# roshanprabhakar/flexflow-train

Hardware: AMD Instinct MI355X
Metric: samples_per_sec_whole_node (higher is better)
Workload: dtype bf16; 1 GPU; model=bert-large, global_batch=128, batch_per_gpu=128, seq_len=512, parallelism=dp1, layers=24, hidden=1024, heads=16, vocab=30522, optimizer=adamw, hipgraph=True, native_replay=True

## Files before the change

csrc/kernels/attention.hip:

```cpp
#include <cstdlib>
#include <type_traits>

#include "kernels.h"
#include "mfma.h"

namespace ffk {

template <class T>
struct TensorViewT {
  T* p;
  int64_t sb, ss, sh;
  __device__ __forceinline__ T* row(int b, int s, int h) const { return p + b * sb + static_cast<int64_t>(s) * ss + h * sh; }
};
using TensorView = TensorViewT<const bf16>;
using OutView = TensorViewT<bf16>;

struct AttnParams {
  TensorView q, k, v, o, dout;
  OutView o_out, dq, dk, dv;
  float* lse;
  float* delta;
  float *dbq, *dbk, *dbv;
  int64_t db_ld;
  int B, H, Sq, Sk;
// ... 164 lines not shown

__device__ __forceinline__ float bfi_sel(unsigned m, float a, float b) {
  float r;
  asm("v_bfi_b32 %0, %1, %2, %3" : "=v"(r) : "v"(m), "v"(a), "v"(b));
  return r;
}
template <int DT>
__device__ __forceinline__ void bias_partial(const f32x16 (&acc)[DT], float mul, float* row, int lane) {
  constexpr int NV = 16 * DT;
  float v[NV];
#pragma unroll
  for (int dt = 0; dt < DT; ++dt)
#pragma unroll
    for (int r = 0; r < 16; ++r) v[dt * 16 + r] = acc[dt][r];
#pragma unroll
  for (int st = 0; st < 5; ++st) {
    const int o = 16 >> st, c = NV >> st;
    const unsigned m = (lane & o) ? ~0u : 0u;
#pragma unroll
    for (int i = 0; i < c / 2; ++i) {
      const float send = bfi_sel(m, v[i], v[i + c / 2]);
      const float keep = bfi_sel(m, v[i + c / 2], v[i]);
      v[i] = keep + __shfl_xor(send, o, 64);
    }
  }
  const int h = lane >> 5;
#pragma unroll
  for (int t = 0; t < NV / 32; ++t) {
    const int k = (lane & 31) * (NV / 32) + t, dt = k >> 4, r = k & 15;
    row[dt * 32 + acc_row(r) + 4 * h] = v[t] * mul;
  }
}

template <int D, bool CAUSAL, bool DROP, bool VARLEN, bool PACKED, bool BIAS, bool GQA = false>
__global__ __launch_bounds__(256, (BIAS && D == 128 ? 1 : 2)) void attn_fwd_kernel(AttnParams P) {
  constexpr int KS = D / 16;
  constexpr int DT = D / 32;
  constexpr int KV = 64;
  constexpr int TILE_BYTES = KV * D * 2;
  __shared__ __attribute__((aligned(16))) unsigned char smem[4 * TILE_BYTES];

  const int lane = threadIdx.x & 63, wave = threadIdx.x >> 6, h = lane >> 5;
  int bh = blockIdx.x, qb = gridDim.y - 1 - blockIdx.y;
  if (!CAUSAL) attn_head_block(bh, qb);
  const int b = bh / P.H, hh = bh % P.H;
  const int hk = kv_head<GQA>(P, hh);
  [[maybe_unused]] int pn = b, ps = 0, plen = 0;
  if constexpr (PACKED) {
    const Segment sg = segment_of(P, b);
    pn = sg.n, ps = sg.start, plen = sg.len;
  }
  const int q_blk = qb * 128;
  const int qw = q_blk + wave * 32;
  const int q = qw + (lane & 31);
  const bool q_ok = PACKED ? q < plen : q < P.Sq;
  const int Skl = PACKED ? plen : key_len<VARLEN>(P, b);
  [[maybe_unused]] const int Sql = PACKED ? plen : query_len<VARLEN>(P, b);
  const bool q_live = VARLEN ? q < Sql : q_ok;
  if constexpr (VARLEN) {
    if (q_blk >= Sql) {
      if constexpr (!PACKED) {
        if (q_ok) {
          store_zero_rows<D>(P.o_out.row(b, q, hh), h);
          if (h == 0) P.lse[static_cast<int64_t>(bh) * P.Sq + q] = -INFINITY;
        }
      }
// ... 624 lines not shown
            }
            dv[dt] = mfma32(da, pf, dv[dt]);
            dk[dt] = mfma32(qa, sf, dk[dt]);
          }
        }
        prio_lo(P);
      }
    }
    if (has_next) {
      unsigned char* nxt = smem + ((t + 1 - t0) & 1) * STAGE;
      ql.store(nxt);
      dl.store(nxt + TILE_BYTES);
      park_scalars(nxt);
    }
    __syncthreads();
    if constexpr (GQA) tq = tq_n, hq = hq_n;
  }
  float vmul = 1.f;
  if constexpr (DROP) vmul = P.drop_rs;
  if (P.db_ld) {
    if (kw < P.Sk) {
      const int64_t roff = (static_cast<int64_t>(b) * ((P.Sk + 31) / 32) + kw / 32) * P.db_ld + hh * D;
      if (P.dbk) bias_partial<DT>(dk, P.scale, P.dbk + roff, lane);
      if (P.dbv) bias_partial<DT>(dv, vmul, P.dbv + roff, lane);
    }
  } else {
    if (P.dbk) bias_colsum<DT>(dk, P.scale, P.dbk + hh * D, lane);
    if (P.dbv) bias_colsum<DT>(dv, vmul, P.dbv + hh * D, lane);
  }
  store_rows16<DT>(P.dk.row(pn, ps + key, hh), dk, P.scale, h, k_st);
  store_rows16<DT>(P.dv.row(pn, ps + key, hh), dv, vmul, h, k_st);
}

__global__ __launch_bounds__(512, 1) void attn_bwd_onepass_kernel(AttnParams P, float* __restrict__ ws) {
  constexpr int D = 64, KS = D / 16, DT = D / 32, QT = 64, KB = 256, NT = 512;
  constexpr int TILE_BYTES = QT * D * 2;
  constexpr int STAGE = 2 * TILE_BYTES + 2 * QT * 4;
  constexpr int KIMG_BYTES = KB * D * 2, DS_BYTES = KB * QT * 2;
  __shared__ __attribute__((aligned(16))) unsigned char smem[2 * STAGE + KIMG_BYTES + 2 * DS_BYTES];
  unsigned char* const Kimg = smem + 2 * STAGE;
  unsigned char* const dSimg = Kimg + KIMG_BYTES;
  const int lane = threadIdx.x & 63, wave = __builtin_amdgcn_readfirstlane(threadIdx.x >> 6), h = lane >> 5;
  const int bh = blockIdx.x, b = bh / P.H, hh = bh % P.H;
  const int n_q_tiles = (P.Sq + QT - 1) / QT;
  const int n_kb = (P.Sk + KB - 1) / KB;
  const int w4 = wave & 3, dq_par = wave >> 2, dq_q = (w4 & 1) * 32, dq_d = (w4 >> 1) * 32;
  const int srow = threadIdx.x >> 3, sch = threadIdx.x & 7;

  TileLoader<D, QT, NT> ql, dl, ol;
  float nls = 0.f;
  bool nok = false;
  auto fetch = [&](int q0) {
    ql.load(P.q, b, hh, q0, P.Sq);
    dl.load(P.dout, b, hh, q0, P.Sq);
    ol.load(P.o, b, hh, q0, P.Sq);
    nok = q0 + srow < P.Sq;
    if (nok && sch == 0) nls = P.lse[static_cast<int64_t>(bh) * P.Sq + q0 + srow];
  };
  auto park = [&](unsigned char* stage) {
    ql.store(stage);
    dl.store(stage + TILE_BYTES);
    float part = 0.f;
#pragma unroll
    for (int e = 0; e < 8; ++e) part += bf2f(ol.reg[0][e]) * bf2f(dl.reg[0][e]);
#pragma unroll
    for (int o = 1; o < 8; o <<= 1) part += __shfl_xor(part, o, 64);
    if (sch == 0) {
      float* ls = reinterpret_cast<float*>(stage + 2 * TILE_BYTES);
      ls[srow] = nok ? -nls * P.inv_scale_log2 : -INFINITY;
      ls[QT + srow] = -part;
    }
  };

  for (int kb = 0; kb < n_kb; ++kb) {
    const int k_blk = kb * KB;
    const int kl_ = wave * 32 + (lane & 31);
    const int kw = k_blk + wave * 32, key = k_blk + kl_;
    const bool k_ok = key < P.Sk;
    const bool last_kb = kb == n_kb - 1;
    bf16x8 vf[KS];
#pragma unroll
    for (int ks = 0; ks < KS; ++ks) {
      vf[ks] = k_ok ? *reinterpret_cast<const bf16x8*>(P.v.row(b, key, hh) + ks * 16 + 8 * h) : bf16x8{};
    }
    {
      int r0 = srow;
      asm volatile("" : "+v"(r0));
      const bf16* kp = P.k.row(b, k_blk + r0, hh) + sch * 8;
      bf16x8 kr[KB / 64];
#pragma unroll
      for (int i = 0; i < KB / 64; ++i)
        kr[i] = k_blk + r0 + 64 * i < P.Sk ? *reinterpret_cast<const bf16x8*>(kp + 64 * i * P.k.ss) : bf16x8{};
      int q0 = 0;
      asm volatile("" : "+s"(q0));
      fetch(q0);
#pragma unroll
      for (int i = 0; i < KB / 64; ++i) *reinterpret_cast<bf16x8*>(Kimg + lds_off<D>(r0 + 64 * i, sch)) = kr[i];
    }
    park(smem);
    __syncthreads();

    f32x16 dk[DT], dv[DT];
#pragma unroll
    for (int dt = 0; dt < DT; ++dt) dk[dt] = dv[dt] = f32x16{};

    auto dq_tile = [&](int t) {
      const unsigned char* dS = dSimg + (t & 1) * DS_BYTES;
      float* wp = ws + ((static_cast<int64_t>(bh) * n_q_tiles + t) * 4 + w4) * 1024 + lane * 4;
      f32x16 acc[1] = {f32x16{}};
      const int i16 = lane & 15, colq = 16 * ((lane >> 4) & 1) + 4 * (i16 & 3), ra = 8 * h + (i16 >> 2);
      const int ck = dq_d + colq, cs = dq_q + colq;
      const unsigned char* ka = Kimg + img_off<D * 2>(ra, ck >> 3) + (ck & 7) * 2;
      const unsigned char* kb_ = Kimg + img_off<D * 2>(ra + 4, ck >> 3) + (ck & 7) * 2;
      const unsigned char* sa = dS + img_off<QT * 2>(ra, cs >> 3) + (cs & 7) * 2;
      const unsigned char* sb = dS + img_off<QT * 2>(ra + 4, cs >> 3) + (cs & 7) * 2;
      auto product = [&] {
        prio_hi(P);
#pragma unroll 4
        for (int k0 = 0; k0 < KB; k0 += 16) {
          const int o = k0 * 128;
          acc[0] = mfma32(cat44(lds_tr(ka, o), lds_tr(kb_, o)), cat44(lds_tr(sa, o), lds_tr(sb, o)), acc[0]);
        }
        prio_lo(P);
      };
      if (kb > 0) {
        f32x4 prev[4];
#pragma unroll
        for (int g = 0; g < 4; ++g) prev[g] = *reinterpret_cast<const f32x4*>(wp + g * 256);
        product();
#pragma unroll
        for (int g = 0; g < 4; ++g)
#pragma unroll
          for (int e = 0; e < 4; ++e) acc[0][4 * g + e] += prev[g][e];
      } else {
        product();
      }
      if (last_kb) {
        const int q = t * QT + dq_q + (lane & 31);
        store_rows16<1>(P.dq.row(b, q, hh) + dq_d, acc, P.scale, h, q < P.Sq);
      } else {
#pragma unroll
        for (int g = 0; g < 4; ++g) {
          f32x4 w;
#pragma unroll
          for (int e = 0; e < 4; ++e) w[e] = acc[0][4 * g + e];
          *reinterpret_cast<f32x4*>(wp + g * 256) = w;
        }
      }
    };

    for (int t = 0; t <= n_q_tiles; ++t) {
      const int q0 = t * QT;
      unsigned char* stage = smem + (t & 1) * STAGE;
      const unsigned char* Qt = stage;
      const unsigned char* Dt = stage + TILE_BYTES;
      const float* ls = reinterpret_cast<const float*>(stage + 2 * TILE_BYTES);
      const float* ds = ls + QT;
      unsigned char* dSw = dSimg + (t & 1) * DS_BYTES;
      fetch(q0 + QT);
      const bool need_mask = (q0 + QT > P.Sq) || (kw + 31 >= P.Sk);
      if (t < n_q_tiles) {
#pragma unroll
        for (int qt = 0; qt < 2; ++qt) {
          f32x16 s, dp;
          bf16x8 qa[KS], da[KS], kf[KS], tda[2][DT], tqa[2][DT];
#pragma unroll
          for (int ks = 0; ks < KS; ++ks) {
            const int off = lds_off<D>(qt * 32 + (lane & 31), 2 * ks + h);
            qa[ks] = lds_read16(Qt, off);
            da[ks] = lds_read16(Dt, off);
            kf[ks] = lds_read16(Kimg, lds_off<D>(kl_, 2 * ks + h));
          }
// ... 18 lines not shown
          if (need_mask) {
#pragma unroll
            for (int r = 0; r < 16; ++r) {
              const int qq = q0 + qt * 32 + acc_row(r) + 4 * h;
              float pv = fexp2(s[r] * P.scale_log2);
              if (qq >= P.Sq || !k_ok) pv = 0.f;
              s[r] = pv;
              dp[r] = pv * dp[r];
            }
          } else {
#pragma unroll
            for (int r = 0; r < 16; ++r) {
              const float pv = fexp2(s[r] * P.scale_log2);
              s[r] = pv;
              dp[r] = pv * dp[r];
            }
          }
          prio_hi(P);
#pragma unroll
          for (int st = 0; st < 2; ++st) {
            const bf16x8 pf = acc_to_frag(s, st), sf = acc_to_frag(dp, st);
            if (st == 0) {
#pragma unroll
              for (int dt = 0; dt < DT; ++dt) {
                tda[1][dt] = tr_frag<D>(Dt, qt * 32 + 16, dt, lane);
                tqa[1][dt] = tr_frag<D>(Qt, qt * 32 + 16, dt, lane);
              }
            }
#pragma unroll
            for (int g2 = 0; g2 < 2; ++g2) {
              bf16x4 w;
#pragma unroll
              for (int e = 0; e < 4; ++e) w[e] = sf[4 * g2 + e];
              *reinterpret_cast<bf16x4*>(dSw + img_off<QT * 2>(kl_, qt * 4 + 2 * st + g2) + 8 * h) = w;
            }
#pragma unroll
            for (int dt = 0; dt < DT; ++dt) {
              dv[dt] = mfma32(tda[st][dt], pf, dv[dt]);
              dk[dt] = mfma32(tqa[st][dt], sf, dk[dt]);
            }
          }
          prio_lo(P);
        }
      }
      park(smem + ((t + 1) & 1) * STAGE);
      if (t > 0 && ((t - 1) & 1) == dq_par) dq_tile(t - 1);
      __syncthreads();
    }

    store_rows16<DT>(P.dk.row(b, key, hh), dk, P.scale, h, k_ok);
    store_rows16<DT>(P.dv.row(b, key, hh), dv, 1.f, h, k_ok);
  }
}

__global__ void attn_segment_offsets_kernel(const int32_t* __restrict__ seg_lens, int32_t* __restrict__ seg_off, int N,
                                            int M, int T, int max_seqlen) {
  const int n = blockIdx.x * blockDim.x + threadIdx.x;
  if (n >= N) return;
  int start = 0;
  for (int m = 0; m < M; ++m) {
    const int64_t i = static_cast<int64_t>(n) * M + m;
    const int len = min(max(seg_lens[i], 0), min(max_seqlen, T - start));
    seg_off[2 * i] = start;
    seg_off[2 * i + 1] = len;
    start += len;
  }
}

__global__ __launch_bounds__(256) void attn_pack_tail_kernel(OutView a, OutView b, OutView c, float* __restrict__ lse,
                                                              const int32_t* __restrict__ seg_off, int M, int T, int H,
                                                              int D) {
  constexpr int ROWS = 16;
  const int n = blockIdx.y, row0 = blockIdx.x * ROWS;
  const int64_t last = (static_cast<int64_t>(n) * M + (M - 1)) * 2;
  const int tail = min(max(seg_off[last] + seg_off[last + 1], 0), T);
  if (row0 + ROWS <= tail) return;
  const int cpr = H * (D / 8);
  for (int i = threadIdx.x; i < ROWS * cpr; i += blockDim.x) {
    const int r = row0 + i / cpr, ch = i % cpr, hh = ch / (D / 8), d = (ch % (D / 8)) * 8;
    if (r < tail || r >= T) continue;
    const u32x4t z = {0u, 0u, 0u, 0u};
    if (a.p) *reinterpret_cast<u32x4t*>(a.row(n, r, hh) + d) = z;
    if (b.p) *reinterpret_cast<u32x4t*>(b.row(n, r, hh) + d) = z;
    if (c.p) *reinterpret_cast<u32x4t*>(c.row(n, r, hh) + d) = z;
  }
// ... 142 lines not shown
      constexpr int DD = decltype(d)::value;
      constexpr bool CC = decltype(c)::value, DR = decltype(dr)::value, VL = decltype(vl)::value;
      if constexpr (!DR && !VL) {
        if (P.G > 1) {
          hipLaunchKernelGGL((attn_fwd_kernel<DD, CC, false, false, false, false, true>), grid, block, 0, st, P);
          return;
        }
      }
      if constexpr (VL) {
        if (packed) {
          hipLaunchKernelGGL((attn_fwd_kernel<DD, CC, DR, true, true, false>), grid, block, 0, st, P);
          return;
        }
      }
      if constexpr (!CC && !VL) {
        if (P.bias) {
          hipLaunchKernelGGL((attn_fwd_kernel<DD, false, DR, false, false, true>), grid, block, 0, st, P);
          return;
        }
      }
      hipLaunchKernelGGL((attn_fwd_kernel<DD, CC, DR, VL, false, false>), grid, block, 0, st, P);
    });
  });
  if (packed) launch_pack_tail(P, P.o_out, OutView{}, OutView{}, P.lse, B, D, st);
  FFK_LAUNCH_CHECK("attention_fwd");
}

static bool onepass_eligible(int Sk, int D, bool causal, bool extras) {
  if (D != 64 || causal || Sk > 512 || extras) return false;
  const char* oe = getenv("FFK_ATTN_BWD_ONEPASS");
  return oe ? atoi(oe) != 0 : true;
}

int64_t attention_bwd_workspace(int B, int H, int Sq, int Sk, int D, bool causal, bool dbias, bool varlen) {
  if (!onepass_eligible(Sk, D, causal, dbias || varlen) || Sk <= 256) return 0;
  return static_cast<int64_t>(B) * H * ((Sq + 63) / 64) * 64 * 64;
}

int attention_bwd(const AttnTensors& t, int B, int H, int Sq, int Sk, int D, float scale, bool causal,
                  hipStream_t st, float* ws) {
  AttnParams P = make_params(t, B, H, Sq, Sk, D, scale, causal);
  const bool packed = P.seg_off != nullptr;
  const bool drop = P.drop_thr != 0, varlen = P.kv_lens || P.q_lens || packed;
  if (onepass_eligible(Sk, D, causal, t.dbq || t.dbk || t.dbv || drop || varlen || P.bias || P.G > 1) &&
      (Sk <= 256 || ws)) {
    hipLaunchKernelGGL(attn_bwd_onepass_kernel, dim3(static_cast<unsigned>(B * H)), dim3(512), 0, st, P, ws);
    FFK_LAUNCH_CHECK("attention_bwd");
    return 1;
  }
  const unsigned nq = static_cast<unsigned>((Sq + 127) / 128), nk = static_cast<unsigned>((Sk + 127) / 128);
  const unsigned nbh = static_cast<unsigned>(packed ? B * P.M * H : B * H);
  dim3 gq = causal ? dim3(nbh, nq) : dim3(nq, nbh), gk = causal ? dim3(nbh, nk) : dim3(nk, nbh), block(256);
  with_head(D, causal, [&](auto d, auto c) {
    with_features(drop, varlen, [&](auto dr, auto vl) {
      constexpr int DD = decltype(d)::value;
      constexpr bool CC = decltype(c)::value, DR = decltype(dr)::value, VL = decltype(vl)::value;
      if constexpr (!DR && !VL) {
        if (P.G > 1) {
          const unsigned nkh = static_cast<unsigned>(B * P.Hkv);
          const dim3 gkv = causal ? dim3(nkh, nk) : dim3(nk, nkh);
          hipLaunchKernelGGL((attn_bwd_dq_kernel<DD, CC, false, false, false, false, true>), gq, block, 0, st, P);
          hipLaunchKernelGGL((attn_bwd_dkdv_kernel<DD, CC, false, false, false, false, true>), gkv, block, 0, st, P);
          return;
        }
      }
      if constexpr (VL) {
        if (packed) {
          hipLaunchKernelGGL((attn_bwd_dq_kernel<DD, CC, DR, true, true, false>), gq, block, 0, st, P);
          hipLaunchKernelGGL((attn_bwd_dkdv_kernel<DD, CC, DR, true, true, false>), gk, block, 0, st, P);
          return;
        }
      }
      if constexpr (!CC && !VL) {
        if (P.bias) {
          hipLaunchKernelGGL((attn_bwd_dq_kernel<DD, false, DR, false, false, true>), gq, block, 0, st, P);
          hipLaunchKernelGGL((attn_bwd_dkdv_kernel<DD, false, DR, false, false, true>), gk, block, 0, st, P);
          return;
        }
      }
// ... 11 lines not shown
```

csrc/kernels/bindings.cpp:

```cpp
#include <pybind11/pybind11.h>
#include <pybind11/stl.h>

#include "kernels.h"

namespace py = pybind11;
using namespace ffk;

static inline void* P(uintptr_t p) { return reinterpret_cast<void*>(p); }
static inline float* F(uintptr_t p) { return reinterpret_cast<float*>(p); }
static inline hipStream_t S(uintptr_t s) { return reinterpret_cast<hipStream_t>(s); }

static AttnTensors::T tview(const py::tuple& t) {
  AttnTensors::T r;
  if (t.size() != 4) throw std::invalid_argument("attention tensor view must be (ptr, sb, ss, sh)");
  r.p = P(t[0].cast<uintptr_t>());
  r.sb = t[1].cast<int64_t>();
  r.ss = t[2].cast<int64_t>();
  r.sh = t[3].cast<int64_t>();
  return r;
}

static void set_packed(AttnTensors& t, uintptr_t seg_off, int seg_M, int seg_T) {
  if (!seg_off) return;
  t.seg_offsets = reinterpret_cast<const int32_t*>(seg_off);
// ... 156 lines not shown
    set_bias(t, bias);
    set_packed(t, seg_off, seg_M, seg_T);
    t.q = tview(q);
    t.k = tview(k);
    t.v = tview(v);
    t.o = tview(o);
    t.dout = tview(dout);
    t.dq = tview(dq);
    t.dk = tview(dk);
    t.dv = tview(dv);
    t.lse = F(lse);
    t.delta = F(delta);
    t.dbq = F(dbq);
    t.dbk = F(dbk);
    t.dbv = F(dbv);
    t.db_ld = db_ld;
    set_dropout(t, drop_t, seed, seed_dev);
    t.kv_lens = reinterpret_cast<const int32_t*>(kv_lens);
    t.q_lens = reinterpret_cast<const int32_t*>(q_lens);
    return attention_bwd(t, B, H, Sq, Sk, D, scale, causal, S(st), F(ws));
  }, py::arg("q"), py::arg("k"), py::arg("v"), py::arg("o"), py::arg("dout"), py::arg("dq"), py::arg("dk"),
        py::arg("dv"), py::arg("lse"), py::arg("delta"), py::arg("B"), py::arg("H"), py::arg("Sq"), py::arg("Sk"),
        py::arg("D"), py::arg("scale"), py::arg("causal"), py::arg("st"), py::arg("dbq") = 0, py::arg("dbk") = 0,
        py::arg("dbv") = 0, py::arg("db_ld") = 0, py::arg("ws") = 0, py::arg("drop_t") = 0, py::arg("seed") = 0,
        py::arg("seed_dev") = 0, py::arg("kv_lens") = 0, py::arg("q_lens") = 0, py::arg("seg_off") = 0,
        py::arg("seg_M") = 0, py::arg("seg_T") = 0, py::arg("bias") = py::tuple(), py::arg("kv_heads") = 0);
  m.def("attention_segment_offsets", [](uintptr_t seg_lens, uintptr_t seg_off, int N, int M, int T, int max_seqlen,
                                        uintptr_t st) {
    attention_segment_offsets(reinterpret_cast<const int32_t*>(seg_lens), reinterpret_cast<int32_t*>(seg_off), N, M,
                              T, max_seqlen, S(st));
  });
  m.def("attention_bwd_workspace", &attention_bwd_workspace, py::arg("B"), py::arg("H"), py::arg("Sq"),
        py::arg("Sk"), py::arg("D"), py::arg("causal"), py::arg("dbias"), py::arg("varlen") = false);
  m.def("gemm", [](uintptr_t A, uintptr_t B, uintptr_t C, uintptr_t bias, uintptr_t pre, int M, int N, int K,
                   int lda, int ldb, int ldc, bool ta, bool tb, int act, float alpha, float beta, int out_f32,
                   uintptr_t st, int splits, uintptr_t ws) {
    gemm_bf16_ex(P(A), P(B), P(C), P(bias), P(pre), M, N, K, lda, ldb, ldc, ta, tb, act, alpha, beta, out_f32, S(st),
                 splits, F(ws));
  }, py::arg("A"), py::arg("B"), py::arg("C"), py::arg("bias"), py::arg("pre"), py::arg("M"), py::arg("N"),
     py::arg("K"), py::arg("lda"), py::arg("ldb"), py::arg("ldc"), py::arg("ta"), py::arg("tb"), py::arg("act"),
     py::arg("alpha"), py::arg("beta"), py::arg("out_f32"), py::arg("st"), py::arg("splits") = 1,
     py::arg("ws") = 0);
  auto shape = [](const std::vector<int64_t>& v) {
    if (v.size() > 6) throw std::invalid_argument("tensorops: at most 6 dims");
    NdShape s;
    s.nd = static_cast<int>(v.size());
    for (size_t i = 0; i < v.size(); ++i) s.size[i] = v[i];
    return s;
  };
  auto strides = [](const std::vector<int64_t>& v) {
    if (v.size() > 6) throw std::invalid_argument("tensorops: at most 6 dims");
    NdStrides s;
    for (size_t i = 0; i < v.size(); ++i) s.s[i] = v[i];
    return s;
  };
  m.def("binary_nd", [=](int dt, uintptr_t a, uintptr_t b, uintptr_t y, std::vector<int64_t> s,
                         std::vector<int64_t> sa, std::vector<int64_t> sb, int op, uintptr_t st) {
    binary_nd(dt, P(a), P(b), P(y), shape(s), strides(sa), strides(sb), op, S(st));
  });
  m.def("binary_grad_nd", [=](int dt, uintptr_t dy, uintptr_t a, uintptr_t b, uintptr_t g, std::vector<int64_t> s,
                              std::vector<int64_t> sa, std::vector<int64_t> sb, int op, int which, uintptr_t st) {
    binary_grad_nd(dt, P(dy), P(a), P(b), F(g), shape(s), strides(sa), strides(sb), op, which, S(st));
  });
  m.def("sum_to", [=](int dt, uintptr_t full, uintptr_t out, std::vector<int64_t> s, std::vector<int64_t> t,
                      float beta, uintptr_t st) {
    sum_to(dt, F(full), P(out), shape(s), shape(t), beta, S(st));
// ... 236 lines not shown
```

csrc/kernels/kernels.h:

```cpp
#pragma once
#include <hip/hip_runtime.h>
#include <string>
#include <vector>

#include <algorithm>
#include <cstdint>

namespace ffk {

void layernorm_fwd(int dtype, const void* x, const void* res, void* sum_out, const void* gamma, const void* beta,
                   void* y, float* mean, float* rstd, int M, int N, float eps, hipStream_t st);
int layernorm_bwd_grid(int M, int N);
void layernorm_bwd(int dtype, const void* dy, const void* s, const float* mean, const float* rstd,
                   const void* gamma, void* dx, float* dgamma, float* dbeta, float* ws, int M, int N,
                   hipStream_t st, const void* dres = nullptr,
                   float* dsum = nullptr);

void bias_act_fwd(int dtype, const void* x, const void* bias, void* pre, void* y, int64_t M, int64_t N, int op,
                  float alpha, hipStream_t st);
void act_bwd(int dtype, const void* dy, const void* pre, void* dx, int64_t n, int op, float alpha, hipStream_t st);
void colsum_act(int dtype, const void* dy, const void* pre, void* dx, float* dbias, int64_t M, int64_t N, int op,
                float alpha, hipStream_t st);
void dropout_fwd(int dtype, const void* x, void* y, int64_t n, float p, uint64_t seed, hipStream_t st);
void cast(int dtype_in, int dtype_out, const void* x, void* y, int64_t n, hipStream_t st);
// ... 37 lines not shown
  struct T {
    const void* p = nullptr;
    int64_t sb = 0, ss = 0, sh = 0;
  };
  T q, k, v, o, dout, dq, dk, dv;
  float* lse = nullptr;
  float* delta = nullptr;
  float* dbq = nullptr;
  float* dbk = nullptr;
  float* dbv = nullptr;
  int64_t db_ld = 0;
  uint32_t drop_threshold = 0;
  float drop_keep_scale = 1.f;
  uint64_t seed = 0;
  const int64_t* seed_dev = nullptr;
  const int32_t* kv_lens = nullptr;
  const int32_t* q_lens = nullptr;
  const int32_t* seg_offsets = nullptr;
  int seg_M = 0;
  int seg_T = 0;
  struct Bias {
    const float* p = nullptr;
    int64_t sb = 0, sh = 0, sq = 0;
  };
  Bias bias = {};
  int kv_heads = 0;
};
void attention_segment_offsets(const int32_t* seg_lens, int32_t* seg_off, int N, int M, int T, int max_seqlen,
                               hipStream_t st);
void attention_fwd(const AttnTensors& t, int B, int H, int Sq, int Sk, int D, float scale, bool causal,
                   hipStream_t st);
int64_t attention_bwd_workspace(int B, int H, int Sq, int Sk, int D, bool causal, bool dbias,
                                bool varlen = false);
int attention_bwd(const AttnTensors& t, int B, int H, int Sq, int Sk, int D, float scale, bool causal,
                  hipStream_t st, float* ws = nullptr);

void gemm_bf16(const void* A, const void* B, void* C, const void* bias, int M, int N, int K, int lda, int ldb,
               int ldc, bool trans_a, bool trans_b, int act, float alpha, float beta, int out_f32,
               hipStream_t st);
void gemm_bf16_ex(const void* A, const void* B, void* C, const void* bias, void* pre, int M, int N, int K, int lda,
                  int ldb, int ldc, bool trans_a, bool trans_b, int act, float alpha, float beta, int out_f32,
                  hipStream_t st, int splits = 1, float* ws = nullptr);

bool gemm256_supported(int M, int N, int K, int lda, int ldb, bool trans_a, bool trans_b);
void gemm256_bf16(const void* A, const void* B, void* C, const void* bias, void* pre, int M, int N, int K, int lda,
                  int ldb, int ldc, bool trans_a, bool trans_b, int act, float alpha, float beta, int out_f32,
                  int splits, float* workspace, hipStream_t st);

void splitk_reduce(const float* ws, void* out, int M, int N, int ldc, int S, float beta, int out_f32,
                   hipStream_t st);

struct GemmPParams {
  const void* A = nullptr;
  const void* B = nullptr;
  void* C = nullptr;
  const void* bias = nullptr;
  void* pre = nullptr;
  const void* aux = nullptr;
  float* dbias = nullptr;
  float* workspace = nullptr;
  int M = 0, N = 0, K = 0, lda = 0, ldb = 0, ldc = 0;
  bool trans_a = false, trans_b = false;
  int act = 0;
  bool act_bwd = false;
  float alpha = 1.f, beta = 0.f;
  int out_f32 = 0, splits = 1;
  int dbg = 0;
  int variant = 0;
// ... 178 lines not shown
```

flexflow_train_amd/kernels/__init__.py:

```python
from __future__ import annotations

import collections
import importlib
import math
import os
from typing import Dict, NamedTuple, Optional

import torch

_ext = None
_ext_error: Optional[BaseException] = None
STATS: collections.Counter = collections.Counter()

DT_F32, DT_BF16, DT_F16 = 0, 1, 2
ACT_CODES = {"none": 0, "identity": 0, "relu": 1, "sigmoid": 2, "tanh": 3, "gelu": 4, "elu": 5, "exp": 6}


def _load():
    global _ext, _ext_error
    if _ext is not None or _ext_error is not None:
        return _ext
    try:
        _ext = importlib.import_module("flexflow_train_amd._ffkernels")
    except BaseException as e:
# ... 553 lines not shown
    Sk = k.shape[1]
    Hkv = _attn_gqa(q, k, v, dropout_p, kv_lens, q_lens, seg_lens, bias, dbias)
    if Hkv:
        if k.shape != (B, Sk, Hkv, D) or v.shape != (B, Sk, Hkv, D):
            raise ValueError("attention: q/k/v shape mismatch")
        for name, t, shp in (("o", o, (B, Sq, H, D)), ("do", do, (B, Sq, H, D)), ("dq", dq, (B, Sq, H, D)),
                             ("dk", dk, (B, Sk, Hkv, D)), ("dv", dv, (B, Sk, Hkv, D))):
            if tuple(t.shape) != shp:
                raise ValueError(f"attention_bwd: {name} has shape {tuple(t.shape)}, expected {shp}"
                                 + (f" (grouped-query: dk / dv take the Hkv = {Hkv} K / V heads)"
                                    if name in ("dk", "dv") else ""))
        if lse.shape != (B, H, Sq) or lse.dtype != torch.float32 or not lse.is_contiguous():
            raise ValueError("attention_bwd: bad lse")
        delta = torch.empty(B, H, Sq, device=q.device, dtype=torch.float32)
        sc = float(scale) if scale is not None else 1.0 / math.sqrt(D)
        path = ext().attention_bwd(_view4(q), _view4(k), _view4(v), _view4(o), _view4(do), _view4(dq), _view4(dk),
                                   _view4(dv), lse.data_ptr(), delta.data_ptr(), B, H, Sq, Sk, D, sc, bool(causal),
                                   _stream(), kv_heads=Hkv)
        STATS["attention_gqa"] += 1
        STATS["attention_bwd"] += 1
        return path
    bview, bkeep = _attn_bias(bias, q, Sq, Sk, causal, kv_lens, q_lens, seg_lens, dbias)
    pk = None
    if seg_lens is not None:
        pk = _attn_packed(seg_lens, max_seqlen, seg_offsets, q, k, v, kv_lens, q_lens, dbias)
    for name, t, shp in (("o", o, (B, Sq, H, D)), ("do", do, (B, Sq, H, D)), ("dq", dq, (B, Sq, H, D)),
                         ("dk", dk, (B, Sk, H, D)), ("dv", dv, (B, Sk, H, D))):
        if tuple(t.shape) != shp:
            raise ValueError(f"attention_bwd: {name} has shape {tuple(t.shape)}, expected {shp}")
    if lse.shape != (B, H, Sq) or lse.dtype != torch.float32 or not lse.is_contiguous():
        raise ValueError("attention_bwd: bad lse")
    delta = torch.empty(B, H, Sq, device=q.device, dtype=torch.float32)
    sc = float(scale) if scale is not None else 1.0 / math.sqrt(D)
    dbs, ld, slab = [0, 0, 0], 0, None
    HD = H * D
    if dbias is not None:
        for t in dbias:
            if t is not None:
                _check(t, "dbias", torch.float32, HD)
        if dbias_atomic:
            dbs = [t.data_ptr() if t is not None else 0 for t in dbias]
        else:
            nq, nk = (Sq + 31) // 32, (Sk + 31) // 32
            slab = torch.empty(B * max(nq, nk), 3 * HD, device=q.device, dtype=torch.float32)
            ld = 3 * HD
            dbs = [slab.data_ptr() + 4 * i * HD if t is not None else 0 for i, t in enumerate(dbias)]
    if pk is not None:
        drop = _attn_dropout_args(dropout_p, seed, seed_dev, q, pk[3], pk[3])
        ext().attention_bwd(_view4(q), _view4(k), _view4(v), _view4(o), _view4(do), _view4(dq), _view4(dk),
                            _view4(dv), lse.data_ptr(), delta.data_ptr(), B, H, pk[3], pk[3], D, sc, bool(causal),
                            _stream(), 0, 0, 0, 0, 0, *drop, 0, 0, pk[0], pk[1], pk[2])
        STATS["attention_bwd"] += 1
        return 0
    drop = _attn_dropout_args(dropout_p, seed, seed_dev, q, Sq, Sk)
    lens = _attn_kv_lens(kv_lens, q)
    qlens = _attn_q_lens(q_lens, q)
    n_ws = 0 if drop[0] or bview else ext().attention_bwd_workspace(B, H, Sq, Sk, D, bool(causal),
                                                                     dbias is not None, bool(lens or qlens))
    ws = torch.empty(n_ws, device=q.device, dtype=torch.float32) if n_ws else None
    path = ext().attention_bwd(_view4(q), _view4(k), _view4(v), _view4(o), _view4(do), _view4(dq), _view4(dk),
                               _view4(dv), lse.data_ptr(), delta.data_ptr(), B, H, Sq, Sk, D, sc, bool(causal),
                               _stream(), *dbs, ld, _p(ws), *drop, lens, **({"q_lens": qlens} if qlens else {}),
                               **({"bias": bview} if bview else {}))
    if path == 1:
        STATS["attention_bwd_onepass"] += 1
    if slab is not None:
        rows = (B * nq, B * nk, B * nk)
        for i, t in enumerate(dbias):
            if t is not None:
                t.add_(slab[:rows[i], i * HD:(i + 1) * HD].sum(0))
    STATS["attention_bwd"] += 1
    return path


def gemm(a, b, trans_a=False, trans_b=False, bias=None, act="none", alpha=1.0, beta=0.0, out=None,
         out_dtype=None, pre=None, splits=1):
    if a.dtype != torch.bfloat16 or b.dtype != torch.bfloat16:
        raise ValueError("gemm: operands must be bf16")
    if a.dim() != 2 or b.dim() != 2 or a.stride(1) != 1 or b.stride(1) != 1:
        raise ValueError("gemm: operands must be 2-D with unit inner stride")
    M, K = (a.shape[1], a.shape[0]) if trans_a else (a.shape[0], a.shape[1])
    Kb, N = (b.shape[1], b.shape[0]) if trans_b else (b.shape[0], b.shape[1])
    if K != Kb:
        raise ValueError(f"gemm: inner dims differ ({K} vs {Kb})")
    dt = out_dtype or (out.dtype if out is not None else torch.bfloat16)
    if out is None:
        out = torch.empty(M, N, device=a.device, dtype=dt)
    if out.shape != (M, N) or out.stride(1) != 1:
        raise ValueError("gemm: bad output")
    if bias is not None:
        _check(bias, "bias", torch.bfloat16, N)
    if pre is not None:
        _check(pre, "pre", torch.bfloat16, M * N)
        if _ld2d(out) != N:
            raise ValueError("gemm: pre needs a dense output")
    splits = max(1, min(int(splits), (K + 63) // 64))
    if splits > 1 and (N % 4 or out.stride(0) % 4):
        splits = 1
    ws = _splitk_ws(a.device, splits * M * N) if splits > 1 else None
    ext().gemm(a.data_ptr(), b.data_ptr(), out.data_ptr(), _p(bias), _p(pre), M, N, K, a.stride(0), b.stride(0),
               out.stride(0), bool(trans_a), bool(trans_b), ACT_CODES[act], float(alpha), float(beta),
               int(out.dtype == torch.float32), _stream(), splits, _p(ws))
    STATS["gemm"] += 1
    if splits > 1:
        STATS["gemm_splitk"] += 1
# ... 1310 lines not shown
```

flexflow_train_amd/ops/attention.py:

```python
from __future__ import annotations

import math
import os
import warnings

import torch

from .. import kernels as K
from ..parallel import sequence as SP
from .base import OpContext, OpImpl, acc_grad, register
from .gemm import matmul, wgrad_matmul

_FUSED_DBIAS = os.environ.get("FF_ATTN_FUSED_DBIAS", "0") == "1"


def _dims(ctx: OpContext, q, k, v, W):
    H_local = W.shape[-1] if W.dim() == 2 else None
    E = int(ctx.a("embed_dim"))
    H = int(ctx.a("num_heads"))
    kd = int(ctx.a("kdim") or 0) or E // H
    vd = int(ctx.a("vdim") or 0) or E // H
    Hl = H // max(1, ctx.input_copy_degree)
    if H_local is not None:
        Hl = H_local
    return E, Hl, kd, vd, q.shape[-1], k.shape[-1], v.shape[-1]


def _split_weights(W, E, Hl, kd, vd, Eq, Ek, Ev):
    flat = W.reshape(-1)
    if Eq == Ek == Ev and kd == vd:
        n_qkv = Eq * 3 * Hl * kd
        Wqkv = flat[:n_qkv].view(Eq, 3 * Hl * kd)
        Wo = flat[n_qkv:n_qkv + Hl * vd * E].view(Hl * vd, E)
        W3 = Wqkv.view(Eq, 3, Hl * kd)
        return {"qkv": Wqkv, "o": Wo, "q": W3[:, 0], "k": W3[:, 1], "v": W3[:, 2]}
    o0 = 0
    Wq = flat[o0:o0 + Eq * Hl * kd].view(Eq, Hl * kd)
    o0 += Eq * Hl * kd
    Wk = flat[o0:o0 + Ek * Hl * kd].view(Ek, Hl * kd)
    o0 += Ek * Hl * kd
    Wv = flat[o0:o0 + Ev * Hl * vd].view(Ev, Hl * vd)
    o0 += Ev * Hl * vd
    Wo = flat[o0:o0 + Hl * vd * E].view(Hl * vd, E)
    return {"q": Wq, "k": Wk, "v": Wv, "o": Wo}


# ... 341 lines not shown
        if db_out is not None:
            if gpu:
                K.colsum_act(dout, None, "none", db_out, write_dx=False)
            else:
                acc_grad(db_out, dout.float().sum(0))
        wbeta = ctx.extra.get("wgrad_beta", [1.0])[0]
        if dW_views is not None:
            if gpu:
                wgrad_matmul(ctx, o2, dout, dW_views["o"], wbeta)
            else:
                acc_grad(dW_views["o"], o2.float().t() @ dout.float())
        do = matmul(dout, ws["o"], trans_b=True) if gpu else dout @ ws["o"].to(dout.dtype).t()
        do4 = do.view(B, Sq, Hl, vd)
        if self_attn:
            qkv = proj
            qkv5 = qkv.view(B, Sq, 3, Hl, kd)
            q, k, v = qkv5[:, :, 0], qkv5[:, :, 1], qkv5[:, :, 2]
        else:
            q, k, v = proj
        if isinstance(lse, tuple):
            dq_, dk_, dv_ = SP.sp_attention_bwd(do4, lse[1], causal, scale, ctx.extra["seq_group"])
            if self_attn:
                dproj = torch.stack([dq_, dk_, dv_], dim=2).reshape(B * Sq, 3 * Hl * kd)
            else:
                dq, dk, dv = dq_, dk_, dv_
        elif lse is not None:
            if self_attn:
                dproj = torch.empty_like(qkv)
                d5 = dproj.view(B, Sq, 3, Hl, kd)
                dq, dk, dv = d5[:, :, 0], d5[:, :, 1], d5[:, :, 2]
            else:
                dq, dk, dv = torch.empty_like(q), torch.empty_like(k), torch.empty_like(v)
            fused_db = None
            if _FUSED_DBIAS and seg is None and self_attn and db_in is not None and kd == vd \
                    and db_in.dtype == torch.float32 and db_in.is_contiguous():
                dbf = db_in.reshape(-1)
                n = Hl * kd
                fused_db = (dbf[:n], dbf[n:2 * n], dbf[2 * n:3 * n])
            kw = dict(dropout_p=drop[0], seed=drop[1], seed_dev=drop[2]) if drop else {}
            if seg is not None:
                kw.update(seg_lens=seg, max_seqlen=max_seqlen, seg_offsets=seg_off)
            K.attention_bwd(q, k, v, o, lse, do4, dq, dk, dv, causal=causal, scale=scale, dbias=fused_db,
                            kv_lens=lens, q_lens=qlens, **kw)
            if fused_db is not None:
                db_in = None
        else:
            qf, kf, vf = (t.detach().float().requires_grad_(True) for t in (q, k, v))
            if seg is not None:
                ref = _torch_packed_attention(qf, kf, vf, causal, scale, seg, max_seqlen,
                                              _fallback_mask(drop, B * seg.shape[1], Hl, max_seqlen, max_seqlen))
            else:
                ref = _torch_attention(qf, kf, vf, causal, scale, _fallback_mask(drop, B, Hl, Sq, Sk), lens, qlens)
            ref.float().backward(do4.float())
            dq, dk, dv = (t.grad.to(do.dtype) for t in (qf, kf, vf))
            if self_attn:
                dproj = torch.stack([dq, dk, dv], dim=2).reshape(B * Sq, 3 * Hl * kd)
        dx_q = dx_k = dx_v = None
        if self_attn:
            d2 = dproj.view(B * Sq, 3 * Hl * kd)
            if db_in is not None:
                if gpu:
                    K.colsum_act(d2, None, "none", db_in.reshape(-1), write_dx=False)
                else:
                    acc_grad(db_in, d2.float().sum(0))
            if dW_views is not None:
                if gpu:
                    wgrad_matmul(ctx, x2, d2, dW_views["qkv"], wbeta)
                else:
# ... 130 lines not shown
```

Before: 872.7 samples/s.

## Fuse QKV bias-gradient reduction into one-pass attention backward kernel by default

```diff
diff --git a/csrc/kernels/attention.hip b/csrc/kernels/attention.hip
--- a/csrc/kernels/attention.hip
+++ b/csrc/kernels/attention.hip
@@ -220,6 +220,24 @@
   }
 }
 
+__device__ __forceinline__ float piece_colsum(const f32x16& acc, int lane) {
+  float v[16];
+#pragma unroll
+  for (int r = 0; r < 16; ++r) v[r] = acc[r];
+#pragma unroll
+  for (int st = 0; st < 4; ++st) {
+    const int o = 16 >> st, c = 16 >> st;
+    const unsigned m = (lane & o) ? ~0u : 0u;
+#pragma unroll
+    for (int i = 0; i < c / 2; ++i) {
+      const float send = bfi_sel(m, v[i], v[i + c / 2]);
+      const float keep = bfi_sel(m, v[i + c / 2], v[i]);
+      v[i] = keep + __shfl_xor(send, o, 64);
+    }
+  }
+  return v[0] + __shfl_xor(v[0], 1, 64);
+}
+
 template <int D, bool CAUSAL, bool DROP, bool VARLEN, bool PACKED, bool BIAS, bool GQA = false>
 __global__ __launch_bounds__(256, (BIAS && D == 128 ? 1 : 2)) void attn_fwd_kernel(AttnParams P) {
   constexpr int KS = D / 16;
@@ -910,20 +928,31 @@
   store_rows16<DT>(P.dv.row(pn, ps + key, hh), dv, vmul, h, k_st);
 }
 
+template <bool DBIAS>
 __global__ __launch_bounds__(512, 1) void attn_bwd_onepass_kernel(AttnParams P, float* __restrict__ ws) {
   constexpr int D = 64, KS = D / 16, DT = D / 32, QT = 64, KB = 256, NT = 512;
   constexpr int TILE_BYTES = QT * D * 2;
   constexpr int STAGE = 2 * TILE_BYTES + 2 * QT * 4;
   constexpr int KIMG_BYTES = KB * D * 2, DS_BYTES = KB * QT * 2;
-  __shared__ __attribute__((aligned(16))) unsigned char smem[2 * STAGE + KIMG_BYTES + 2 * DS_BYTES];
+  constexpr int DB_KV = 2 * 2 * 8 * 64, DB_BYTES = DBIAS ? (DB_KV + 8 * 32) * 4 : 0;
+  __shared__ __attribute__((aligned(16))) unsigned char smem[2 * STAGE + KIMG_BYTES + 2 * DS_BYTES + DB_BYTES];
   unsigned char* const Kimg = smem + 2 * STAGE;
   unsigned char* const dSimg = Kimg + KIMG_BYTES;
+  [[maybe_unused]] float* const dbp = reinterpret_cast<float*>(dSimg + 2 * DS_BYTES);
   const int lane = threadIdx.x & 63, wave = __builtin_amdgcn_readfirstlane(threadIdx.x >> 6), h = lane >> 5;
   const int bh = blockIdx.x, b = bh / P.H, hh = bh % P.H;
   const int n_q_tiles = (P.Sq + QT - 1) / QT;
   const int n_kb = (P.Sk + KB - 1) / KB;
   const int w4 = wave & 3, dq_par = wave >> 2, dq_q = (w4 & 1) * 32, dq_d = (w4 >> 1) * 32;
   const int srow = threadIdx.x >> 3, sch = threadIdx.x & 7;
+  [[maybe_unused]] auto dq_sum = [&]() -> float* {
+    int l = lane;
+    asm volatile("" : "+v"(l));
+    return (l & 1) ? nullptr : dbp + DB_KV + wave * 32 + acc_row((l & 31) >> 1) + 4 * (l >> 5);
+  };
+  if constexpr (DBIAS) {
+    if (float* w = dq_sum()) *w = 0.f;
+  }
 
   TileLoader<D, QT, NT> ql, dl, ol;
   float nls = 0.f;
@@ -990,8 +1019,9 @@
       const int ck = dq_d + colq, cs = dq_q + colq;
       const unsigned char* ka = Kimg + img_off<D * 2>(ra, ck >> 3) + (ck & 7) * 2;
       const unsigned char* kb_ = Kimg + img_off<D * 2>(ra + 4, ck >> 3) + (ck & 7) * 2;
-      const unsigned char* sa = dS + img_off<QT * 2>(ra, cs >> 3) + (cs & 7) * 2;
-      const unsigned char* sb = dS + img_off<QT * 2>(ra + 4, cs >> 3) + (cs & 7) * 2;
+      const int sh8 = ((cs & 7) * 2) ^ ((ra & 1) << 3);
+      const unsigned char* sa = dS + img_off<QT * 2>(ra, cs >> 3) + sh8;
+      const unsigned char* sb = dS + img_off<QT * 2>(ra + 4, cs >> 3) + sh8;
       auto product = [&] {
         prio_hi(P);
 #pragma unroll 4
@@ -1016,6 +1046,10 @@
       if (last_kb) {
         const int q = t * QT + dq_q + (lane & 31);
         store_rows16<1>(P.dq.row(b, q, hh) + dq_d, acc, P.scale, h, q < P.Sq);
+        if constexpr (DBIAS) {
+          const float cs = piece_colsum(acc[0], lane);
+          if (float* w = dq_sum()) *w += cs;
+        }
       } else {
 #pragma unroll
         for (int g = 0; g < 4; ++g) {
@@ -1100,7 +1134,7 @@
               bf16x4 w;
 #pragma unroll
               for (int e = 0; e < 4; ++e) w[e] = sf[4 * g2 + e];
-              *reinterpret_cast<bf16x4*>(dSw + img_off<QT * 2>(kl_, qt * 4 + 2 * st + g2) + 8 * h) = w;
+              *reinterpret_cast<bf16x4*>(dSw + img_off<QT * 2>(kl_, qt * 4 + 2 * st + g2) + 8 * (h ^ (lane & 1))) = w;
             }
 #pragma unroll
             for (int dt = 0; dt < DT; ++dt) {
@@ -1118,7 +1152,74 @@
 
     store_rows16<DT>(P.dk.row(b, key, hh), dk, P.scale, h, k_ok);
     store_rows16<DT>(P.dv.row(b, key, hh), dv, 1.f, h, k_ok);
-  }
+    if constexpr (DBIAS) {
+      float* part = dbp + (kb * 16 + wave) * 64;
+      bias_partial<DT>(dk, P.scale, part, lane);
+      bias_partial<DT>(dv, 1.f, part + 8 * 64, lane);
+    }
+  }
+  if constexpr (DBIAS) {
+    __syncthreads();
+    if (threadIdx.x < 192) {
+      const int which = wave, c = lane;
+      float s = 0.f;
+      if (which == 0) {
+#pragma unroll
+        for (int w = 0; w < 4; ++w) s += dbp[DB_KV + ((w >> 1) * 4 + 2 * (c >> 5) + (w & 1)) * 32 + (c & 31)];
+        s *= P.scale;
+      } else {
+        for (int i = 0; i < n_kb; ++i)
+#pragma unroll
+          for (int w = 0; w < 8; ++w) s += dbp[((i * 2 + which - 1) * 8 + w) * 64 + c];
+      }
+      float* const out = which == 0 ? P.dbq : which == 1 ? P.dbk : P.dbv;
+      if (out) out[b * P.db_ld + hh * D + c] = s;
+    }
+  }
+}
+
+__global__ __launch_bounds__(1024) void attn_dbias_reduce_kernel(const float* __restrict__ sq,
+                                                                  const float* __restrict__ sk,
+                                                                  const float* __restrict__ sv, int64_t ld, int rows_q,
+                                                                  int rows_kv, float* __restrict__ dbq,
+                                                                  float* __restrict__ dbk, float* __restrict__ dbv) {
+  constexpr int G = 16;
+  __shared__ float part[G][64];
+  const int which = blockIdx.y;
+  float* const out = which == 0 ? dbq : which == 1 ? dbk : dbv;
+  if (!out) return;
+  const float* p = (which == 0 ? sq : which == 1 ? sk : sv) + blockIdx.x * 64 + (threadIdx.x & 63);
+  const int rows = which == 0 ? rows_q : rows_kv, g = threadIdx.x >> 6;
+  float a0 = 0.f, a1 = 0.f, a2 = 0.f, a3 = 0.f;
+  int r = g;
+  for (; r + 3 * G < rows; r += 4 * G) {
+    a0 += p[r * ld];
+    a1 += p[(r + G) * ld];
+    a2 += p[(r + 2 * G) * ld];
+    a3 += p[(r + 3 * G) * ld];
+  }
+  for (; r < rows; r += G) a0 += p[r * ld];
+  part[g][threadIdx.x & 63] = (a0 + a1) + (a2 + a3);
+  __syncthreads();
+  if (g == 0) {
+    const int c = threadIdx.x;
+    float s = 0.f;
+#pragma unroll
+    for (int i = 0; i < G; ++i) s += part[i][c];
+    out[blockIdx.x * 64 + c] += s;
+  }
+}
+
+void attention_dbias_reduce(const float* sq, const float* sk, const float* sv, int64_t ld, int rows_q, int rows_kv,
+                            float* dbq, float* dbk, float* dbv, int HD, hipStream_t st) {
+  if (HD <= 0 || HD % 64 || ld < HD || rows_q < 0 || rows_kv < 0)
+    throw std::invalid_argument("attention_dbias_reduce: H * D must be a positive multiple of 64 and ld >= H * D");
+  if ((dbq && !sq) || (dbk && !sk) || (dbv && !sv))
+    throw std::invalid_argument("attention_dbias_reduce: an output without its slab");
+  if (!dbq && !dbk && !dbv) return;
+  hipLaunchKernelGGL(attn_dbias_reduce_kernel, dim3(static_cast<unsigned>(HD / 64), 3), dim3(1024), 0, st, sq, sk, sv,
+                     ld, rows_q, rows_kv, dbq, dbk, dbv);
+  FFK_LAUNCH_CHECK("attention_dbias_reduce");
 }
 
 __global__ void attn_segment_offsets_kernel(const int32_t* __restrict__ seg_lens, int32_t* __restrict__ seg_off, int N,
@@ -1327,6 +1428,8 @@
   return oe ? atoi(oe) != 0 : true;
 }
 
+bool attention_bwd_onepass(int Sk, int D, bool causal, bool extras) { return onepass_eligible(Sk, D, causal, extras); }
+
 int64_t attention_bwd_workspace(int B, int H, int Sq, int Sk, int D, bool causal, bool dbias, bool varlen) {
   if (!onepass_eligible(Sk, D, causal, dbias || varlen) || Sk <= 256) return 0;
   return static_cast<int64_t>(B) * H * ((Sq + 63) / 64) * 64 * 64;
@@ -1337,9 +1440,12 @@
   AttnParams P = make_params(t, B, H, Sq, Sk, D, scale, causal);
   const bool packed = P.seg_off != nullptr;
   const bool drop = P.drop_thr != 0, varlen = P.kv_lens || P.q_lens || packed;
-  if (onepass_eligible(Sk, D, causal, t.dbq || t.dbk || t.dbv || drop || varlen || P.bias || P.G > 1) &&
+  const bool dbias = t.dbq || t.dbk || t.dbv;
+  if (onepass_eligible(Sk, D, causal, (dbias && P.db_ld <= 0) || drop || varlen || P.bias || P.G > 1) &&
       (Sk <= 256 || ws)) {
-    hipLaunchKernelGGL(attn_bwd_onepass_kernel, dim3(static_cast<unsigned>(B * H)), dim3(512), 0, st, P, ws);
+    const dim3 grid(static_cast<unsigned>(B * H));
+    if (dbias) hipLaunchKernelGGL(attn_bwd_onepass_kernel<true>, grid, dim3(512), 0, st, P, ws);
+    else hipLaunchKernelGGL(attn_bwd_onepass_kernel<false>, grid, dim3(512), 0, st, P, ws);
     FFK_LAUNCH_CHECK("attention_bwd");
     return 1;
   }
diff --git a/csrc/kernels/bindings.cpp b/csrc/kernels/bindings.cpp
--- a/csrc/kernels/bindings.cpp
+++ b/csrc/kernels/bindings.cpp
@@ -212,6 +212,12 @@
   });
   m.def("attention_bwd_workspace", &attention_bwd_workspace, py::arg("B"), py::arg("H"), py::arg("Sq"),
         py::arg("Sk"), py::arg("D"), py::arg("causal"), py::arg("dbias"), py::arg("varlen") = false);
+  m.def("attention_bwd_onepass", &attention_bwd_onepass, py::arg("Sk"), py::arg("D"), py::arg("causal"),
+        py::arg("extras"));
+  m.def("attention_dbias_reduce", [](uintptr_t sq, uintptr_t sk, uintptr_t sv, int64_t ld, int rows_q, int rows_kv,
+                                     uintptr_t dbq, uintptr_t dbk, uintptr_t dbv, int HD, uintptr_t st) {
+    attention_dbias_reduce(F(sq), F(sk), F(sv), ld, rows_q, rows_kv, F(dbq), F(dbk), F(dbv), HD, S(st));
+  });
   m.def("gemm", [](uintptr_t A, uintptr_t B, uintptr_t C, uintptr_t bias, uintptr_t pre, int M, int N, int K,
                    int lda, int ldb, int ldc, bool ta, bool tb, int act, float alpha, float beta, int out_f32,
                    uintptr_t st, int splits, uintptr_t ws) {
diff --git a/csrc/kernels/kernels.h b/csrc/kernels/kernels.h
--- a/csrc/kernels/kernels.h
+++ b/csrc/kernels/kernels.h
@@ -93,8 +93,11 @@
                    hipStream_t st);
 int64_t attention_bwd_workspace(int B, int H, int Sq, int Sk, int D, bool causal, bool dbias,
                                 bool varlen = false);
+bool attention_bwd_onepass(int Sk, int D, bool causal, bool extras);
 int attention_bwd(const AttnTensors& t, int B, int H, int Sq, int Sk, int D, float scale, bool causal,
                   hipStream_t st, float* ws = nullptr);
+void attention_dbias_reduce(const float* sq, const float* sk, const float* sv, int64_t ld, int rows_q, int rows_kv,
+                            float* dbq, float* dbk, float* dbv, int HD, hipStream_t st);
 
 void gemm_bf16(const void* A, const void* B, void* C, const void* bias, int M, int N, int K, int lda, int ldb,
                int ldc, bool trans_a, bool trans_b, int act, float alpha, float beta, int out_f32,
diff --git a/flexflow_train_amd/kernels/__init__.py b/flexflow_train_amd/kernels/__init__.py
--- a/flexflow_train_amd/kernels/__init__.py
+++ b/flexflow_train_amd/kernels/__init__.py
@@ -609,19 +609,6 @@
         raise ValueError("attention_bwd: bad lse")
     delta = torch.empty(B, H, Sq, device=q.device, dtype=torch.float32)
     sc = float(scale) if scale is not None else 1.0 / math.sqrt(D)
-    dbs, ld, slab = [0, 0, 0], 0, None
-    HD = H * D
-    if dbias is not None:
-        for t in dbias:
-            if t is not None:
-                _check(t, "dbias", torch.float32, HD)
-        if dbias_atomic:
-            dbs = [t.data_ptr() if t is not None else 0 for t in dbias]
-        else:
-            nq, nk = (Sq + 31) // 32, (Sk + 31) // 32
-            slab = torch.empty(B * max(nq, nk), 3 * HD, device=q.device, dtype=torch.float32)
-            ld = 3 * HD
-            dbs = [slab.data_ptr() + 4 * i * HD if t is not None else 0 for i, t in enumerate(dbias)]
     if pk is not None:
         drop = _attn_dropout_args(dropout_p, seed, seed_dev, q, pk[3], pk[3])
         ext().attention_bwd(_view4(q), _view4(k), _view4(v), _view4(o), _view4(do), _view4(dq), _view4(dk),
@@ -632,8 +619,24 @@
     drop = _attn_dropout_args(dropout_p, seed, seed_dev, q, Sq, Sk)
     lens = _attn_kv_lens(kv_lens, q)
     qlens = _attn_q_lens(q_lens, q)
-    n_ws = 0 if drop[0] or bview else ext().attention_bwd_workspace(B, H, Sq, Sk, D, bool(causal),
-                                                                     dbias is not None, bool(lens or qlens))
+    atomic = dbias is not None and bool(dbias_atomic)
+    dbs, ld, slab = [0, 0, 0], 0, None
+    HD = H * D
+    if dbias is not None:
+        for t in dbias:
+            if t is not None:
+                _check(t, "dbias", torch.float32, HD)
+        if atomic:
+            dbs = [t.data_ptr() if t is not None else 0 for t in dbias]
+        else:
+            extras = bool(drop[0] or bview or lens or qlens)
+            slab_path = int(ext().attention_bwd_onepass(Sk, D, bool(causal), extras))
+            rows = (B, B) if slab_path else (B * ((Sq + 31) // 32), B * ((Sk + 31) // 32))
+            slab = torch.empty(max(rows), 3 * HD, device=q.device, dtype=torch.float32)
+            ld = 3 * HD
+            dbs = [slab.data_ptr() + 4 * i * HD if t is not None else 0 for i, t in enumerate(dbias)]
+    n_ws = 0 if drop[0] or bview else ext().attention_bwd_workspace(B, H, Sq, Sk, D, bool(causal), atomic,
+                                                                     bool(lens or qlens))
     ws = torch.empty(n_ws, device=q.device, dtype=torch.float32) if n_ws else None
     path = ext().attention_bwd(_view4(q), _view4(k), _view4(v), _view4(o), _view4(do), _view4(dq), _view4(dk),
                                _view4(dv), lse.data_ptr(), delta.data_ptr(), B, H, Sq, Sk, D, sc, bool(causal),
@@ -642,12 +645,15 @@
     if path == 1:
         STATS["attention_bwd_onepass"] += 1
     if slab is not None:
-        rows = (B * nq, B * nk, B * nk)
-        for i, t in enumerate(dbias):
-            if t is not None:
-                t.add_(slab[:rows[i], i * HD:(i + 1) * HD].sum(0))
+        if path != slab_path:
+            raise RuntimeError("attention_bwd: the dbias slab was laid out for the other backward path")
+        ext().attention_dbias_reduce(*dbs, ld, rows[0], rows[1], *[_p(t) for t in dbias], HD, _stream())
     STATS["attention_bwd"] += 1
     return path
+
+
+def attention_bwd_onepass(Sk, D, causal=False, extras=False):
+    return bool(ext().attention_bwd_onepass(int(Sk), int(D), bool(causal), bool(extras)))
 
 
 def gemm(a, b, trans_a=False, trans_b=False, bias=None, act="none", alpha=1.0, beta=0.0, out=None,
diff --git a/flexflow_train_amd/ops/attention.py b/flexflow_train_amd/ops/attention.py
--- a/flexflow_train_amd/ops/attention.py
+++ b/flexflow_train_amd/ops/attention.py
@@ -11,7 +11,13 @@
 from .base import OpContext, OpImpl, acc_grad, register
 from .gemm import matmul, wgrad_matmul
 
-_FUSED_DBIAS = os.environ.get("FF_ATTN_FUSED_DBIAS", "0") == "1"
+_FUSED_DBIAS = os.environ.get("FF_ATTN_FUSED_DBIAS", "auto")
+
+
+def _fuse_dbias(Sk, D, causal, extras) -> bool:
+    if _FUSED_DBIAS in ("0", "1"):
+        return _FUSED_DBIAS == "1"
+    return K.attention_bwd_onepass(Sk, D, causal, extras)
 
 
 def _dims(ctx: OpContext, q, k, v, W):
@@ -419,8 +425,9 @@
             else:
                 dq, dk, dv = torch.empty_like(q), torch.empty_like(k), torch.empty_like(v)
             fused_db = None
-            if _FUSED_DBIAS and seg is None and self_attn and db_in is not None and kd == vd \
-                    and db_in.dtype == torch.float32 and db_in.is_contiguous():
+            if seg is None and self_attn and db_in is not None and kd == vd \
+                    and db_in.dtype == torch.float32 and db_in.is_contiguous() \
+                    and _fuse_dbias(Sk, kd, causal, bool(drop and drop[0]) or lens is not None or qlens is not None):
                 dbf = db_in.reshape(-1)
                 n = Hl * kd
                 fused_db = (dbf[:n], dbf[n:2 * n], dbf[2 * n:3 * n])
```

Measured after the change: 878.2 samples/s, median of 6. Within noise of the previous version (+0.6%).
